# yundantianchang/OpenHyperFLOW2D

Measured on AMD Instinct MI355X. Metric: Mcells·iters/sec (whole node) on Wedge15 2000×200, higher is better.
Workload: dtype fp64

## Files before the change

openhyperflow2d_amd/csrc/bind/module.cpp:

```cpp
#include <algorithm>
#include <pybind11/functional.h>
#include <pybind11/numpy.h>
#include <pybind11/pybind11.h>
#include <pybind11/stl.h>

#include <cstring>
#include <iostream>
#include <sstream>

#include "../core/case.hpp"
#include "../core/checkpoint.hpp"
#include "../core/lean_euler.hpp"
#include "../core/postproc.hpp"
#include "../core/solver.hpp"
#include "../hip/chem_mech.hpp"
#include "../hip/chem_fast.hpp"
#include "../hip/chem_rtc.hpp"
#include "../hip/device_solver.hpp"
#include "../hip/numerics.hpp"

namespace py = pybind11;
using namespace hf2d;

namespace {
// ... 487 lines not shown
            const CellRecord& n = c.J.at(i, j);
            double v;
            if (name == "p_total") v = p_asterisk(n);
            else if (name == "T_total") v = T_asterisk(n);
            else if (name == "schlieren") v = schlieren(n);
            else throw std::runtime_error("unknown derived field " + name);
            m(i, j) = v;
          }
        return a;
      })
      .def("save_heat_flux", [](const Case& c, const std::string& px, const std::string& py_) {
        need_whole(c);
        if (!px.empty()) save_x_heat_flux(px, c, c.J);
        if (!py_.empty()) save_y_heat_flux(py_, c, c.J);
      });

  m.def(
      "lean_tile_geom",
      [](int ncols, int ny, int block, int tj, int cpt) {
        const LeanTile T = lean_tile_geom(ncols, ny, block, tj, cpt);
        py::dict d;
        d["TI"] = T.TI;
        d["TJ"] = T.TJ;
        d["W"] = T.W;
        d["NC"] = T.NC;
        d["nbi"] = T.nbi;
        d["nbj"] = T.nbj;
        d["TIh"] = T.TIh;
        d["CPT"] = T.CPT;
        return d;
      },
      py::arg("ncols"), py::arg("ny"), py::arg("block"), py::arg("tj") = 0, py::arg("cpt") = 1,
      "lean tile geometry (lean_euler.hpp LeanTile) of a strip of ncols x ny cells");
  m.def("sk_eligible", [](const Case& c) { std::string w; const int md = sk_eligible(c, &w); return py::make_tuple(md, w); },
        py::arg("case"), "split-kernel specialisation (0 generic, 1 single-gas laminar, 2 single-gas turbulent; reason)");
  m.def("smooth", [](py::array_t<double, py::array::c_style> a, int axis) {
        if (a.ndim() != 2) throw std::runtime_error("smooth: (nx, ny) array expected");
        auto buf = a.mutable_data();
        if (axis == 0) smooth_x(buf, (int)a.shape(0), (int)a.shape(1));
        else smooth_y(buf, (int)a.shape(0), (int)a.shape(1));
      }, py::arg("a"), py::arg("axis"), "SmoothX (axis 0) / SmoothY (axis 1), in place");
  m.def("cond_names", &cond_names, py::arg("CT"), "PrintCond: names of the set CondType2D bits");
  m.def("turb_cond_names", &turb_cond_names, py::arg("TT"), "PrintTurbCond: names of the set TurbulenceCondType2D bits");

  py::class_<SolverBase>(m, "SolverBase")
      .def("run_steps", &SolverBase::run_steps, py::arg("n"), py::arg("want_residual_last") = false,
           py::call_guard<py::gil_scoped_release>())
      .def("advance", [](SolverBase& s, bool want) { s.advance(want); }, py::arg("want_residual") = false)
      .def_property_readonly("phase_times",
                             [](const SolverBase& s) {
                               py::dict d;
                               for (const auto& kv : s.phase_acc)
                                 d[py::str(kv.first)] = py::make_tuple(kv.second.first, kv.second.second);
                               return d;
                             })
      .def("set_comm",
           [](SolverBase& s, int rank, int size, std::function<double(double)> fmin, std::function<double(double)> fsum,
              std::function<int(int)> fmaxi, std::function<py::bytes(py::bytes)> fres,
              std::function<py::object(py::bytes)> fallgather) {
             auto* c = new PyComm();
             c->r = rank;
             c->n = size;
             c->f_min = fmin;
             c->f_sum = fsum;
             c->f_maxi = fmaxi;
             c->f_res = fres;
// ... 368 lines not shown
      .def_readonly("gi0", &DeviceSolver::gi0)
      .def_readonly("gi1", &DeviceSolver::gi1)
      .def_property(
          "lnm_phase_ms",
          [](const DeviceSolver& s) {
            return std::vector<double>(s.lnm_phase_ms, s.lnm_phase_ms + 4);
          },
          [](DeviceSolver& s, const std::vector<double>& v) {
            for (int q = 0; q < 4; q++) s.lnm_phase_ms[q] = q < (int)v.size() ? v[q] : 0.0;
          })
      .def("lnm_trace_fetch", &DeviceSolver::lnm_trace_fetch, py::call_guard<py::gil_scoped_release>())
      .def("comm_rank", &DeviceSolver::comm_rank)
      .def("comm_size", &DeviceSolver::comm_size)
      .def("synchronize", &DeviceSolver::synchronize, py::call_guard<py::gil_scoped_release>())
      .def("autotune", &DeviceSolver::autotune, py::arg("steps") = 120, py::call_guard<py::gil_scoped_release>())
      .def("trace_tile", &DeviceSolver::trace_tile, py::arg("steps") = 20,
           "one phase-traced lean tile step: per workgroup [entry, staged, wave0 computed, reduced, dt atomic done "
           "(s_memrealtime, 100 MHz), HW_ID, XCC_ID, blockIdx]")
      .def_property_readonly("lean_tile_last",
                             [](const DeviceSolver& s) {
                               const DeviceSolver::TileLast& t = s.lean_tile_last;
                               py::dict d;
                               d["nt"] = t.nt;
                               d["cpt"] = t.cpt;
                               d["TI"] = t.TI;
                               d["TJ"] = t.TJ;
                               d["nbi"] = t.nbi;
                               d["nbj"] = t.nbj;
                               d["stagger"] = t.stagger;
                               d["fx"] = t.fx;
                               d["var"] = t.var;
                               d["seen"] = t.seen;
                               d["dt_read"] = t.dt_read;
                               return d;
                             },
                             "geometry and variant (0 plain, 1 outputs, 2 residual) of the last lean tile launch; "
                             "nt == 0 after a step on any other kernel")
      .def("halo_field_count", [](const DeviceSolver& d, int group, bool full) {
        std::vector<real*> f;
        d.halo_fields(group, f, full);
        return (int)f.size();
      }, py::arg("group"), py::arg("full") = false)
      .def_property("lean_plain", [](const DeviceSolver& d) { return d.lean_plain; },
                    [](DeviceSolver& d, bool on) { d.set_lean_plain(on); })
      .def_property_readonly("stream", [](const DeviceSolver& s) { return (uintptr_t)s.stream(); });
}
```

openhyperflow2d_amd/csrc/core/lean_euler.hpp:

```cpp
#pragma once

#include <algorithm>
#include <cstring>

#include "stepkern.hpp"

namespace hf2d {

HF_HD inline bool same_bits(real a, real b) {
  u64 x, y;
  std::memcpy(&x, &a, sizeof x);
  std::memcpy(&y, &b, sizeof y);
  return x == y;
}

enum : uint8_t { LB_DX_OUT = 16, LB_DY_OUT = 32, LB_PLAIN = 64 };

struct LeanSoA {
  long N = 0;
  const real* Sin;
  real* Sout;
  const real* Pin_s;
  real* Pout_s;
  real* beta;
// ... 37 lines not shown
  const long N = L.N;
  switch (k) {
    case I_RHO: return L.Sin[2 * N + at];
    case I_RHOU: return L.Sin[2 * N + at] * u;
    case I_RHOV: return p + L.Sin[2 * N + at] * v;
    case I_RHOE: return (L.Sin[3 * N + at] + p) * v;
    default: return L.Pin_s[(k - 4) * N + at] * v;
  }
}

struct LeanOwn {
  u64 CT = 0;
  uint8_t lb = 0;
  bool filled = false;
  real beta[4 + NCOMP];
  real CP = 0, R = 0, kk = 0;
};

template <int NE = 4 + NCOMP>
HF_HD inline void lean_load_own(const LeanSoA& L, long idx, LeanOwn& o) {
  const long N = L.N;
  o.CT = L.CT[idx];
  o.lb = L.lb[idx];
  o.filled = !has_all(o.CT, CT_SOLID) && has_all(o.CT, CT_NODE_IS_SET);
  if (o.filled) {
#pragma unroll
    for (int k = 0; k < NE; k++) o.beta[k] = L.beta[k * N + idx];
    o.CP = L.CP[idx];
    o.R = L.R[idx];
    o.kk = L.kk[idx];
  }
}

struct LeanIOCommon {
  static constexpr int NE = 4 + NCOMP;
  static constexpr bool skip(int) { return false; }
  HF_HD static constexpr int eq(int k) { return k; }
  const LeanSoA& L;
  long N, idx, iL, iR, iU, iD;
  uint8_t lb = 0;
  bool noslip = false;
  real FT = 0;
  const real* obeta = nullptr;
  bool skip_same = false;
  real sm[NEQ];

  HF_HD LeanIOCommon(const LeanSoA& l, long i) : L(l), N(l.N), idx(i), iL(i), iR(i), iU(i), iD(i) {}
  HF_HD void set_nb_global(int i, int j, int ny, int n1, int n2, int n3, int n4) {
    iL = (long)(i - n1) * ny + j;
    iR = (long)(i + n2) * ny + j;
    iU = idx + n3;
    iD = idx - n4;
  }
  HF_HD real dxL(int k) const { return L.dSdx_in[k * N + iL]; }
  HF_HD real dxR(int k) const { return L.dSdx_in[k * N + iR]; }
  HF_HD real dyU(int k) const { return L.dSdy_in[k * N + iU]; }
  HF_HD real dyD(int k) const { return L.dSdy_in[k * N + iD]; }
  HF_HD real beta(int k) const { return obeta[k]; }
  HF_HD real Src(int) const { return 0.0; }
  HF_HD real SrcAdd(int k) const { return noslip ? L.SrcAdd[k * N + idx] : 0.0; }
  HF_HD void put_S(int k, real v) { sm[k] = v; }
  HF_HD void put_beta(int k, real v) const {
    if (!skip_same || !same_bits(v, obeta[k])) L.beta[k * N + idx] = v;
  }
  HF_HD void put_dS(int k, real a, real b) const {
    if (lb & LB_DX_OUT) L.dSdx_out[k * N + idx] = a;
// ... 194 lines not shown
        c.Tf = L.Tf[idx];
        c.CT = CT;
        c.lam = c.mu = 0.;
        if (SG)
          chemistry_single_gas(c, *P.species);
        else
          chemistry_zeldovich(c, *P.species, P.sm, P.chem_model);
        if (c.R != own.R) io.out_R(c.R);
        if (!io.skip_same || !same_bits(c.CP, own.CP)) io.out_CP(c.CP);
        if (OUT || noslip)
          for (int q = 0; q < NSPEC; q++) L.Y[q * N + idx] = c.Y[q];
      }
    }
  }
  for (int k = 0; k < NE; k++) io.out_S(k, s[k]);
  io.out_UVP(U, V, p);
  if (OUT) {
    L.Tout[idx] = Tg;
    L.kk[idx] = kk;
  }
  return dt_local;
}

constexpr int LEAN_TILE_FIELDS = 13;
constexpr int LEAN_TILE_FIELDS_SG = 7;
inline int lean_tile_fields(bool sg) { return sg ? LEAN_TILE_FIELDS_SG : LEAN_TILE_FIELDS; }
constexpr int LEAN_TILE_MIN_TJ = 8;

struct LeanTile {
  int TI, TJ, W, NC, nbi, nbj;
  int TIh;
  int CPT;
  int ne = 1;
};

inline LeanTile lean_tile_geom(int ncols, int ny, int block, int tj = 0, int cpt = 1) {
  LeanTile T;
  if (tj > 0) {
    T.TJ = std::min(std::max(tj, LEAN_TILE_MIN_TJ), std::min(block, ny));
  } else if (ny <= 32) {
    T.TJ = ny;
  } else {
    double best = -1;
    T.TJ = 32;
    for (int c = 16; c <= 32; c++) {
      const int nj = (ny + c - 1) / c;
      const double eff = (double)((block / c) * c) / block * (double)ny / (nj * c);
      if (eff > best + 1e-12) {
        best = eff;
        T.TJ = c;
      }
    }
  }
  T.CPT = cpt;
  T.TIh = block / T.TJ;
  T.TI = T.TIh * cpt;
  T.W = T.TJ + 2;
  T.NC = (T.TI + 2) * T.W;
  T.nbi = (ncols + T.TI - 1) / T.TI;
  T.nbj = (ny + T.TJ - 1) / T.TJ;
  return T;
}

template <bool SG = false>
HF_HD inline void lean_tile_stage(const StepParams& P, const LeanSoA& L, const LeanTile& T, int i0, int j0,
                                  real* lds, int t, int nthreads) {
// ... 146 lines not shown
```

openhyperflow2d_amd/csrc/hip/dev_common.hpp:

```cpp
#pragma once

#include <hip/hip_runtime.h>

#include "../core/lean_euler.hpp"
#include "../core/stepkern.hpp"

namespace hf2d {

struct DevScalars {
  unsigned long long dt_bits[3];
  double iter[3];
  double beta_min[3], cfl_min[3];
  double time_part;
  int neg_T;
  int pad;
  double dt_val[3];
  unsigned hot_cnt[3];
  unsigned hot_cnt2[3];
  unsigned long long dt_lag[3];
  alignas(128) unsigned long long dt_sh[3][16][16];
};
constexpr int DT_SHARDS = 16;

__device__ inline double bits_to_d(unsigned long long b) { return __longlong_as_double((long long)b); }
// ... 43 lines not shown
  else if (lane == DT_SHARDS) b = sc->dt_bits[slot];
#pragma unroll
  for (int off = 1; off < 32; off <<= 1) b = dt_bits_min(b, (unsigned long long)__shfl_xor((long long)b, off, 64));
  return bits_to_d((unsigned long long)__shfl((long long)b, 0, 64));
}

__device__ inline double dt_cur(const StepParams& P, const DevScalars* sc, int slot) {
  return __builtin_expect(P.lag_dt != 0, 0) ? bits_to_d(sc->dt_lag[slot]) : dt_get(sc, slot);
}
__device__ inline double dt_cur_tile(const StepParams& P, const DevScalars* sc, int slot) {
  if (__builtin_expect(P.lag_dt != 0, 0)) return bits_to_d(sc->dt_lag[slot]);
  if (P.dt_read == 2) return bits_to_d(sc->dt_bits[slot]);
  if (P.dt_read == 1) return dt_get_wave(sc, slot);
  return dt_get(sc, slot);
}
__device__ inline void lag_head(const StepParams& P, DevScalars* sc, int slot, int slot_next, double fold = 1.0) {
  if (P.lag_dt) {
    const double m = dt_get(sc, slot);
    sc->dt_lag[slot_next] = d_to_bits(fold < m ? fold : m);
  }
}

__device__ inline void apply_dt(StepParams& P, const DevScalars* sc, int slot, bool tile = false) {
  const double dt = tile ? dt_cur_tile(P, sc, slot) : dt_cur(P, sc, slot);
  P.dt = dt;
  P.dtdx = dt / P.dx;
  P.dtdy = dt / P.dy;
  if (P.scen) {
    P.beta_min = sc->beta_min[slot];
    P.CFL_min = sc->cfl_min[slot];
  }
}

__device__ inline void scenario_next(const StepParams& P, DevScalars* sc, int slot, int slot_next) {
  const double it = sc->iter[slot] + 1.0;
  sc->iter[slot_next] = it;
  if (P.scen) {
    const real bs = table_eval(P.scen->beta, it), cs = table_eval(P.scen->cfl, it);
    sc->beta_min[slot_next] = (bs < P.scen->beta0) ? bs : P.scen->beta0;
    sc->cfl_min[slot_next] = (cs < P.scen->CFL) ? cs : P.scen->CFL;
  }
}

constexpr int BLOCK = 256;
constexpr int WAVE = 64;

__device__ inline void shfl_merge(ResidualPack& r, int off) {
#pragma unroll
  for (int k = 0; k < NEQ; k++) {
    EqResidual o;
    o.dd_max = __shfl_xor(r.eq[k].dd_max, off, WAVE);
    o.i = __shfl_xor(r.eq[k].i, off, WAVE);
    o.j = __shfl_xor(r.eq[k].j, off, WAVE);
    o.rms = __shfl_xor(r.eq[k].rms, off, WAVE);
    o.sum_div = __shfl_xor(r.eq[k].sum_div, off, WAVE);
    o.count = __shfl_xor(r.eq[k].count, off, WAVE);
    EqResidual& f = r.eq[k];
    const bool later = (o.i > f.i) || (o.i == f.i && o.j > f.j);
    if (o.dd_max > f.dd_max || (o.dd_max == f.dd_max && later)) {
      f.dd_max = o.dd_max;
      f.i = o.i;
      f.j = o.j;
    }
    f.rms += o.rms;
    f.sum_div += o.sum_div;
    f.count += o.count;
// ... 6 lines not shown
  if (b >= q * NUM_XCD) return b;
  return (b % NUM_XCD) * q + b / NUM_XCD;
}

constexpr int MAX_HALO_FIELDS = 128;
struct ColList {
  real* f[MAX_HALO_FIELDS];
  unsigned char o[MAX_HALO_FIELDS] = {};
  int nf;
};
constexpr long P2P_SPIN_LIMIT = 1L << 26;
constexpr int P2P_THREADS = 512;

__device__ inline unsigned long long p2p_acquire(const unsigned long long* f) {
  return __hip_atomic_load(f, __ATOMIC_ACQUIRE, __HIP_MEMORY_SCOPE_SYSTEM);
}

__device__ inline double p2p_load(const double* p) {
  return __longlong_as_double((long long)__hip_atomic_load((const unsigned long long*)p, __ATOMIC_RELAXED,
                                                           __HIP_MEMORY_SCOPE_SYSTEM));
}
__device__ inline float p2p_load(const float* p) {
  return __int_as_float((int)__hip_atomic_load((const unsigned*)p, __ATOMIC_RELAXED, __HIP_MEMORY_SCOPE_SYSTEM));
}

__device__ inline void p2p_store(double* p, double v) {
  __hip_atomic_store((unsigned long long*)p, (unsigned long long)__double_as_longlong(v), __ATOMIC_RELAXED,
                     __HIP_MEMORY_SCOPE_SYSTEM);
}
__device__ inline void p2p_store(float* p, float v) {
  __hip_atomic_store((unsigned*)p, (unsigned)__float_as_int(v), __ATOMIC_RELAXED, __HIP_MEMORY_SCOPE_SYSTEM);
}
__device__ inline void vm_drain() { asm volatile("s_waitcnt vmcnt(0)" ::: "memory"); }

__device__ inline unsigned long long rt_clock() { return __builtin_amdgcn_s_memrealtime(); }
constexpr int FX_DONE_STRIDE = 32;
constexpr int FX_TRACE_N = 64, FX_TRACE_W = 8;
constexpr unsigned FX_COUNT1_MAX = 512;
constexpr int FX_DONE_WORDS = (DT_SHARDS + 1) * FX_DONE_STRIDE + 2 * FX_TRACE_N * FX_TRACE_W;
struct FusedX {
  real* peer_recv_l;
  real* peer_recv_r;
  const real* my_recv;
  unsigned long long* const* peer_flags;
  double* const* peer_dtr;
  const unsigned long long* my_flags;
  const double* my_dtr;
  unsigned long long* seq;
  unsigned* done;
  long cap;
  int rank, nranks, sides, on;
  int defer;
  int skip;
  int edge_first;
  int count1;
};

__device__ inline double wave_min(double v) {
#pragma unroll
  for (int off = 1; off < WAVE; off <<= 1) v = fmin(v, __shfl_xor(v, off, WAVE));
  return v;
}
template <class Need>
__device__ inline double p2p_wait_wave(const FusedX& x, unsigned long long target, DevScalars* sc, Need need,
                                       bool fold, int par, bool* ok) {
  const int lane = (int)(threadIdx.x & (WAVE - 1));
// ... 164 lines not shown
```

openhyperflow2d_amd/csrc/hip/device_solver.hpp:

```cpp
#pragma once

#include <algorithm>
#include <chrono>
#include <condition_variable>
#include <cstdlib>
#include <memory>
#include <mutex>
#include <string>
#include <thread>
#include <vector>

#include "../core/solver.hpp"
#include "device_knobs.hpp"

namespace hf2d {

struct LnmArrays;
struct LeanTile;

bool gpu_available();

struct LocalGroup {
  explicit LocalGroup(int n_)
      : n(n_), send_l(n_), send_r(n_), dt_src(n_, nullptr), vals(n_), packs(n_), blobs(n_) {
    const char* j = std::getenv("HF2D_LOCAL_JITTER_US");
    jitter_us = j ? std::max(0, std::atoi(j)) : 0;
  }
  int n;
  std::mutex mu;
  std::condition_variable cv;
  int arrived = 0;
  long gen = 0;
  int jitter_us = 0;
  unsigned long long jitter_state = 0x9E3779B97F4A7C15ull;
  void jitter() {
    unsigned long long x;
    {
      std::lock_guard<std::mutex> lk(mu);
      jitter_state ^= jitter_state << 13;
      jitter_state ^= jitter_state >> 7;
      jitter_state ^= jitter_state << 17;
      x = jitter_state;
    }
    std::this_thread::sleep_for(std::chrono::microseconds((long)(x % (unsigned long long)jitter_us)));
  }
  std::vector<real*> send_l, send_r;
  std::vector<const unsigned long long*> dt_src;
  std::vector<double> vals;
  std::vector<ResidualPack> packs;
  std::vector<std::string> blobs;
  void barrier() {
    if (jitter_us > 0) jitter();
    std::unique_lock<std::mutex> lk(mu);
// ... 67 lines not shown
  void halo_fields(int group, std::vector<real*>& f, bool full = false) const;
  void halo_fields(int group, std::vector<real*>& f, std::vector<unsigned char>& o, bool full) const;
  std::string p2p_probe();
  std::vector<unsigned long long> fx_trace();
  static bool p2p_probe_ok(const std::vector<std::string>& blobs, int rank, std::string* why);
  void p2p_fallback();

  std::vector<unsigned long long> lnm_trace_fetch();
  void set_lean_plain(bool on);
  void lean_materialize();
  void lns_materialize();
  void flush_pending();

  bool lean_ok = false;
  std::string lean_why;
  bool lean_sg_ok = false;
  bool lean_has_cauchy_x = true;
  bool any_cauchy_x = true;
  bool sgl_ok = false;
  std::string sgl_why;
  int sk_mode = 0;
  bool lns_ok = false;
  std::string lns_why;
  int lns_turb = 2;
  bool lnm_ok = false;
  std::string lnm_why;
  int lnm_turb = 0;
  bool chem_fast_ok = false;
  bool chem_rtc_ok = false;
  std::string chem_rtc_why;
  std::string chem_kernel_used;
  struct TileLast {
    int nt = 0, cpt = 0, TI = 0, TJ = 0, nbi = 0, nbj = 0, stagger = 0, fx = 0, var = 0, seen = 0, dt_read = 0;
  };
  TileLast lean_tile_last;

  long nstep = 0;
  long lns_steps = 0, lnm_steps = 0;
  long lns_fx_steps = 0;
  long lns_prologue_steps = 0;
  long p2p_mwg_exchanges = 0;
  long overlap_steps = 0;
  long graph_launches = 0;
  long graph_captures = 0;
  double lnm_phase_ms[4] = {0, 0, 0, 0};

  HostArrays h;
  int dev = 0;
  int gi0 = 0, gi1 = 0, l_off = 0;
  int abuf = 0, dsbuf = 0, pbuf = 0, sbuf = 0;
  int cbuf = 0;
  int lean_state = 0;
  int lns_state = 0;
  bool lean_plain = false;
  bool lean_T_stored = true;
  int lns_prev_mu_t = -1;
  double time_offset = 0.0, last_dev_time = 0.0;
  bool dt_word_valid = false;
  unsigned long long* tile_trace = nullptr;
  std::vector<long> probe_idx_host;
  std::vector<real> probe_buf_host;
  int probe_gen = 0;
  long probe_cap = 0;
  std::vector<long> probe_rec_idx;
  bool stats_on = false;
  bool stats_armed = false;
// ... 69 lines not shown
```

openhyperflow2d_amd/csrc/hip/lean_tile.hpp:

```cpp
#pragma once

#include "../core/lean_euler.hpp"
#include "dev_common.hpp"

namespace hf2d {

__device__ __forceinline__ void host_mirror_tail(const StepParams& P, DevScalars* sc, int slot_next) {
  const int lane = (int)(threadIdx.x & (WAVE - 1));
  vm_drain();
  int last = 0;
  if (lane == 0) {
    const unsigned G = gridDim.x, sh = blockIdx.x % DT_SHARDS;
    const unsigned pop = (G - sh + DT_SHARDS - 1) / DT_SHARDS, nsh = G < DT_SHARDS ? G : DT_SHARDS;
    unsigned* cs = P.host_done + sh * FX_DONE_STRIDE;
    unsigned* ct = P.host_done + DT_SHARDS * FX_DONE_STRIDE;
    if (__hip_atomic_fetch_add(cs, 1u, __ATOMIC_RELAXED, __HIP_MEMORY_SCOPE_AGENT) == pop - 1) {
      __hip_atomic_store(cs, 0u, __ATOMIC_RELAXED, __HIP_MEMORY_SCOPE_AGENT);
      if (__hip_atomic_fetch_add(ct, 1u, __ATOMIC_RELAXED, __HIP_MEMORY_SCOPE_AGENT) == nsh - 1) {
        __hip_atomic_store(ct, 0u, __ATOMIC_RELAXED, __HIP_MEMORY_SCOPE_AGENT);
        last = 1;
      }
    }
  }
  if (!__shfl(last, 0, WAVE)) return;
  unsigned long long b = ~0ull;
  if (lane < DT_SHARDS) b = __hip_atomic_load(&sc->dt_sh[slot_next][lane][0], __ATOMIC_RELAXED, __HIP_MEMORY_SCOPE_AGENT);
  if (lane == DT_SHARDS) b = __hip_atomic_load(&sc->dt_bits[slot_next], __ATOMIC_RELAXED, __HIP_MEMORY_SCOPE_AGENT);
  if (P.dt_fold) {
    unsigned long long m = b;
#pragma unroll
    for (int off = 1; off < 32; off <<= 1) m = dt_bits_min(m, (unsigned long long)__shfl_xor((long long)m, off, WAVE));
    m = (unsigned long long)__shfl((long long)m, 0, WAVE);
    if (lane == DT_SHARDS) {
      b = m;
      __hip_atomic_store(&sc->dt_bits[slot_next], m, __ATOMIC_RELAXED, __HIP_MEMORY_SCOPE_AGENT);
    }
  }
  if (!P.host_sc) return;
  DevScalars* h = static_cast<DevScalars*>(P.host_sc);
  if (lane <= DT_SHARDS) (lane < DT_SHARDS ? h->dt_sh[slot_next][lane][0] : h->dt_bits[slot_next]) = b;
  if (lane == DT_SHARDS + 1) h->neg_T = __hip_atomic_load(&sc->neg_T, __ATOMIC_RELAXED, __HIP_MEMORY_SCOPE_AGENT);
}
__device__ __forceinline__ void host_mirror_head(const StepParams& P, const DevScalars* sc, int slot_next) {
  DevScalars* h = static_cast<DevScalars*>(P.host_sc);
  h->time_part = sc->time_part;
  h->dt_lag[slot_next] = sc->dt_lag[slot_next];
}

constexpr int TILE_TRACE_WORDS = 8;
#ifndef HF2D_TILE_STAGGER
#define HF2D_TILE_STAGGER 1
#endif
constexpr int LDS_PER_CU = 160 * 1024;


template <bool RES, bool OUT, bool SG, int CPT, bool FX = false, bool TR = false, int NT = BLOCK>
__device__ __forceinline__ void lean_tile_body(StepParams& P, const LeanSoA& L, const LeanTile& T, DevScalars* sc,
                                               int slot, int slot_next, int serial, ResidualPack* partials,
                                               const FusedX& X = FusedX{}, unsigned long long* trace = nullptr,
                                               int part = 0) {
  extern __shared__ real lds[];
  unsigned long long tr[5];
  if (TR) tr[0] = rt_clock();
  if (HF2D_TILE_STAGGER && SG && CPT == 2 && !FX && NT == BLOCK && P.stagger != 0) {
    const unsigned r = blockIdx.x / (unsigned)P.stagger_wgs;
    if (r < 4 && (P.stagger < 0 || r > 0)) {
      const unsigned long long d = P.stagger > 0 ? (unsigned long long)r * (unsigned)P.stagger
                                                 : (unsigned long long)blockIdx.x * (unsigned)(-P.stagger) /
                                                       (unsigned)P.stagger_wgs;
      const unsigned long long t0 = rt_clock();
      while (rt_clock() - t0 < d) __builtin_amdgcn_s_sleep(2);
    }
  }
  const unsigned b = (FX && X.edge_first) ? tile_edge_first(xcd_remap(blockIdx.x, gridDim.x), T)
                                          : tile_of_part(xcd_remap(blockIdx.x, gridDim.x), part, T);
  unsigned long long seq_prev = 0;
  if (FX) seq_prev = *X.seq;
  apply_dt(P, sc, slot, true);
  if (b == 0 && threadIdx.x < WAVE) {
    double fold = 1.0;
    if (FX && X.defer && P.lag_dt && seq_prev > 0) {
      bool ok;
      fold = p2p_wait_wave(X, seq_prev, sc, [](int) { return true; }, true, (int)(seq_prev & 1), &ok);
    }
    if (threadIdx.x == 0) {
      dt_reset(sc, slot_reset(slot));
      lag_head(P, sc, slot, slot_next, fold);
      sc->dt_bits[slot] = d_to_bits(P.dt);
      sc->time_part += P.dt;
      scenario_next(P, sc, slot, slot_next);
      if (OUT && !RES && !FX && P.host_sc) host_mirror_head(P, sc, slot_next);
    }
  }
  int i[CPT], j[CPT], c[CPT], i0, j0;
  bool mine[CPT];
  LeanOwn own[CPT];
#pragma unroll
  for (int q = 0; q < CPT; q++) {
    mine[q] = lean_tile_cell(P, T, (int)b, (int)threadIdx.x, &i[q], &j[q], &c[q], &i0, &j0, q);
    if (mine[q]) lean_load_own<TileIO<SG>::NE>(L, (long)i[q] * P.ny + j[q], own[q]);
  }
  if (!FX || seq_prev == 0 || (X.skip & 4) || (i0 - 1 > P.i0 - 1 && i0 + T.TI < P.i1)) {
    lean_tile_stage<SG>(P, L, T, i0, j0, lds, threadIdx.x, NT);
  } else {
    constexpr int NF = SG ? LEAN_TILE_FIELDS_SG : LEAN_TILE_FIELDS;
    const int pp = (int)(seq_prev & 1);
    const real* mbL = X.my_recv + ((long)pp * 2) * X.cap;
    const real* mbR = X.my_recv + ((long)pp * 2 + 1) * X.cap;
    const long N = L.N;
    constexpr int NS = SG ? 4 : 4 + NCOMP;
    constexpr int FU = SG ? 4 : 10;
    for (int c = threadIdx.x; c < T.NC; c += NT) {
      const int ii = c / T.W - 1, jj = c - (ii + 1) * T.W - 1;
      const bool xh = ii < 0 || ii >= T.TI, yh = jj < 0 || jj >= T.TJ;
      const int gi = i0 + ii, gj = j0 + jj;
      if ((xh && yh) || gi < 0 || gi >= P.nx || gj < 0 || gj >= P.ny) continue;
      const bool gl = (X.sides & 1) && gi == P.i0 - 1, gr = (X.sides & 2) && gi == P.i1;
      if (gl || gr) {
        const real* mb = gl ? mbL : mbR;
#pragma unroll
        for (int f = 0; f < NF; f++) lds[f * T.NC + c] = p2p_load(mb + (long)f * P.ny + gj);
        continue;
      }
      const long g = (long)gi * P.ny + gj;
#pragma unroll
      for (int f = 0; f < NS; f++) lds[f * T.NC + c] = L.Sin[f * N + g];
      if (!SG)
#pragma unroll
        for (int f = 0; f < NCOMP; f++) lds[(4 + NCOMP + f) * T.NC + c] = L.Pin_s[f * N + g];
      lds[FU * T.NC + c] = L.Uin[g];
      lds[(FU + 1) * T.NC + c] = L.Vin[g];
      lds[(FU + 2) * T.NC + c] = L.Pin[g];
    }
  }
  __syncthreads();
  if (TR) tr[1] = rt_clock();
  ResidualPack r;
  if (RES) {
    residual_reset(r);
#pragma unroll
    for (int k = 0; k < NEQ; k++) r.eq[k].i = r.eq[k].j = -1;
  }
  double dtl = 1.0;
  int neg = 0;
#pragma unroll
  for (int q = 0; q < CPT; q++) {
    if (mine[q]) {
      TileIO<SG> io(L, (long)i[q] * P.ny + j[q], lds, T.NC, T.W, c[q]);
      dtl = fmin(dtl, lean_cell<RES, OUT>(P, L, io, own[q], i[q], j[q], r, &neg));
      if (FX) {
        const bool pl = (X.sides & 1) && i[q] == P.i0, pr = (X.sides & 2) && i[q] == P.i1 - 1;
        if ((pl || pr) && !(X.skip & 2)) {
          constexpr int NF = SG ? LEAN_TILE_FIELDS_SG : LEAN_TILE_FIELDS;
          constexpr int NS = SG ? 4 : 4 + NCOMP;
          const int pn = (int)((seq_prev + 1) & 1);
          real* mb = pl ? X.peer_recv_l + ((long)pn * 2 + 1) * X.cap : X.peer_recv_r + ((long)pn * 2) * X.cap;
          const long N = L.N, g = (long)i[q] * P.ny + j[q];
          real v[NF];
#pragma unroll
          for (int f = 0; f < NS; f++) v[f] = L.Sout[f * N + g];
          if (!SG)
#pragma unroll
            for (int f = 0; f < NCOMP; f++) v[4 + NCOMP + f] = L.Pout_s[f * N + g];
          v[NF - 3] = L.Uout[g];
          v[NF - 2] = L.Vout[g];
          v[NF - 1] = L.Pout[g];
#pragma unroll
          for (int f = 0; f < NF; f++) p2p_store(mb + (long)f * P.ny + j[q], v[f]);
// ... 84 lines not shown
```

openhyperflow2d_amd/csrc/hip/step_tile.hip:

```cpp

#include "device_impl.hpp"
#include "lean_tile.hpp"

namespace hf2d {

template <bool RES, bool FROMG>
__global__ __launch_bounds__(BLOCK) void hf2d_lean_euler(StepParams P, LeanSoA L, long c0, long c1, DevScalars* sc,
                                                          int slot, int slot_next, int serial,
                                                          ResidualPack* partials) {
  apply_dt(P, sc, slot);
  const unsigned b = xcd_remap(blockIdx.x, gridDim.x);
  const long g = (long)b * BLOCK + threadIdx.x;
  if (g == 0) {
    dt_reset(sc, slot_reset(slot));
    lag_head(P, sc, slot, slot_next);
    sc->dt_bits[slot] = d_to_bits(P.dt);
    sc->time_part += P.dt;
    scenario_next(P, sc, slot, slot_next);
  }
  const long c = c0 + g;
  ResidualPack r;
  if (RES) {
    residual_reset(r);
#pragma unroll
// ... 45 lines not shown
     {hf2d_lean_tile<false, false, true, 0, 2>, hf2d_lean_tile<false, true, true, 0, 2>,
      hf2d_lean_tile<true, true, true, 0, 2>}}};
static const TileFxK kTileFx[2][2][3] = {
    {{hf2d_lean_tile_fx<false, false, false, 1>, hf2d_lean_tile_fx<false, true, false, 1>,
      hf2d_lean_tile_fx<true, true, false, 1>},
     {hf2d_lean_tile_fx<false, false, false, 2>, hf2d_lean_tile_fx<false, true, false, 2>,
      hf2d_lean_tile_fx<true, true, false, 2>}},
    {{hf2d_lean_tile_fx<false, false, true, 1>, hf2d_lean_tile_fx<false, true, true, 1>,
      hf2d_lean_tile_fx<true, true, true, 1>},
     {hf2d_lean_tile_fx<false, false, true, 2>, hf2d_lean_tile_fx<false, true, true, 2>,
      hf2d_lean_tile_fx<true, true, true, 2>}}};
static const TileTrK kTileTr[2][2] = {{hf2d_lean_tile_tr<false, 1>, hf2d_lean_tile_tr<false, 2>},
                                      {hf2d_lean_tile_tr<true, 1>, hf2d_lean_tile_tr<true, 2>}};
#define HF2D_NT_ROW(K, NT, CPT) {K<false, false, NT, CPT>, K<false, true, NT, CPT>, K<true, true, NT, CPT>}
static const TileK kTileNt[2][2][3] = {{HF2D_NT_ROW(hf2d_lean_tile_nt, 128, 1), HF2D_NT_ROW(hf2d_lean_tile_nt, 128, 2)},
                                       {HF2D_NT_ROW(hf2d_lean_tile_nt, 64, 1), HF2D_NT_ROW(hf2d_lean_tile_nt, 64, 2)}};
static const TileFxK kTileFxNt[2][2][3] = {
    {HF2D_NT_ROW(hf2d_lean_tile_fx_nt, 128, 1), HF2D_NT_ROW(hf2d_lean_tile_fx_nt, 128, 2)},
    {HF2D_NT_ROW(hf2d_lean_tile_fx_nt, 64, 1), HF2D_NT_ROW(hf2d_lean_tile_fx_nt, 64, 2)}};
#undef HF2D_NT_ROW
static const TileTrK kTileTrNt[2][2] = {{hf2d_lean_tile_tr_nt<128, 1>, hf2d_lean_tile_tr_nt<128, 2>},
                                        {hf2d_lean_tile_tr_nt<64, 1>, hf2d_lean_tile_tr_nt<64, 2>}};
inline int tile_nt(int want, bool sg) { return sg && (want == 128 || want == 64) ? want : BLOCK; }
inline TileK tile_kernel(int nt, bool sg, int cpt, int var) {
  return nt == BLOCK ? kTile[sg][cpt - 1][var] : kTileNt[nt == 128 ? 0 : 1][cpt - 1][var];
}
inline TileFxK tile_fx_kernel(int nt, bool sg, int cpt, int var) {
  return nt == BLOCK ? kTileFx[sg][cpt - 1][var] : kTileFxNt[nt == 128 ? 0 : 1][cpt - 1][var];
}
inline TileTrK tile_tr_kernel(int nt, bool sg, int cpt) {
  return nt == BLOCK ? kTileTr[sg][cpt - 1] : kTileTrNt[nt == 128 ? 0 : 1][cpt - 1];
}

using LeanEulerK = void (*)(StepParams, LeanSoA, long, long, DevScalars*, int, int, int, ResidualPack*);
static const LeanEulerK kLeanEuler[2][2] = {{hf2d_lean_euler<false, false>, hf2d_lean_euler<false, true>},
                                            {hf2d_lean_euler<true, false>, hf2d_lean_euler<true, true>}};

void DeviceSolver::lean_materialize() {
  p2p_complete();
  Impl& m = *impl;
  StepParams P = make_params(last_iter + iter);
  P.nx = h.nx;
  P.ny = h.ny;
  LeanSoA L = m.lean_view(h, sbuf, abuf, dsbuf, pbuf, false);
  SoA g = m.view(h, sbuf, abuf, dsbuf, pbuf);
  const unsigned nb = (unsigned)((h.N + BLOCK - 1) / BLOCK);
  hipLaunchKernelGGL(hf2d_lean_materialize, dim3(nb), dim3(BLOCK), 0, m.stream, P, L, g, 0L, h.N);
  HIP_CHECK(hipGetLastError());
  lean_state = 0;
}

DeviceSolver::StepDone DeviceSolver::step_tile(StepCtx& c) {
  Impl& m = *impl;
  hipStream_t st = m.stream;
  StepParams& P = c.P;
  const bool want_res = c.want_res;
  const int slot = c.slot, slot_next = c.slot_next, serial = c.serial;
  LeanSoA L = m.lean_view(h, sbuf, abuf, dsbuf, pbuf, false);
  P.skip_same = tile_skip_same ? 1 : 0;
  P.dt_read = dt_read_mode == 1 ? 1 : 0;
  const bool sg = lean_sg && lean_sg_ok;
  const int nt = tile_nt(lean_nt, sg);
  int cpt = lean_cpt == 2 ? 2 : 1;
  if (cpt == 2 && nt == BLOCK) {
    const LeanTile T2 = lean_tile_geom(P.i1 - P.i0, P.ny, BLOCK, lean_tj, 2);
    if ((long)T2.nbi * T2.nbj < 2L * cu_count) cpt = 1;
  }
  const LeanTile T = lean_tile_geom(P.i1 - P.i0, P.ny, nt, lean_tj, cpt);
  const unsigned ntile = (unsigned)(T.nbi * T.nbj);
  size_t shmem = (size_t)lean_tile_fields(sg) * T.NC * sizeof(real);
  if (lean_wgcu > 0)
    shmem = std::max(shmem, (size_t)((LDS_PER_CU / lean_wgcu - 1024) & ~255));
  const bool rec_out = (probe_cap > 0 || stats_on) && !sg && P.chem_model != NO_REACTIONS;
  const bool out = step_outputs || want_res || rec_out;
  P.stagger_wgs = cu_count > 0 ? cu_count : 256;
  P.stagger = ntile <= 4u * (unsigned)P.stagger_wgs && nt == BLOCK ? tile_stagger : 0;
  const bool fx_step = m.p2p.on && p2p_fuse && !lean_has_cauchy_x;
  FusedX X = fx_step ? fused_args() : FusedX{};
  X.defer = fx_step && P.lag_dt ? 1 : 0;
  lean_tile_last.nt = nt;
  lean_tile_last.cpt = cpt;
  lean_tile_last.TI = T.TI;
  lean_tile_last.TJ = T.TJ;
  lean_tile_last.nbi = T.nbi;
  lean_tile_last.nbj = T.nbj;
  lean_tile_last.stagger = HF2D_TILE_STAGGER && sg && cpt == 2 && !fx_step && nt == BLOCK ? P.stagger : 0;
  lean_tile_last.fx = fx_step ? 1 : 0;
  lean_tile_last.seen = c.tile_prev.nt == nt && c.tile_prev.cpt == cpt ? c.tile_prev.seen : 0;
  const bool split = comm_overlap && !fx_step && !m.p2p.on && (m.comm || m.local) && m.nranks > 1 &&
                     !want_res && !out && !tile_trace;
  if (split) {
    lean_tile_last.seen |= 1;
    lean_T_stored = false;
    overlap_streams();
    const bool parts = T.nbi >= 3;
    const unsigned ne = parts ? (unsigned)(2 * T.nbj) : ntile, ni = parts ? (unsigned)((T.nbi - 2) * T.nbj) : 0u;
    const TileK pk = tile_kernel(nt, sg, cpt, 0);
    hipLaunchKernelGGL(pk, dim3(ne), dim3(nt), shmem, st, P, L, T, m.sc, slot, slot_next, serial, m.partials,
                       parts ? 1 : 0);
    HIP_CHECK(hipGetLastError());
    sbuf = 1 - sbuf;
    dsbuf = 1 - dsbuf;
    pbuf = 1 - pbuf;
    HIP_CHECK(hipEventRecord(m.ev_edge, st));
    if (ni > 0)
      hipLaunchKernelGGL(pk, dim3(ni), dim3(nt), shmem, st, P, L, T, m.sc, slot, slot_next, serial, m.partials,
                         2);
    HIP_CHECK(hipGetLastError());
    overlap_exchange(CpuSolver::HALO_LEAN, slot_next);
    return {ntile, nt / WAVE, true};
  }
  const int var = want_res ? 2 : out ? 1 : 0;
  lean_tile_last.var = var;
  lean_tile_last.seen |= 1 << var;
  lean_T_stored = var != 0;
  if (tile_trace && var == 0 && !fx_step)
    hipLaunchKernelGGL(tile_tr_kernel(nt, sg, cpt), dim3(ntile), dim3(nt), shmem, st, P, L, T, m.sc, slot, slot_next,
                       serial, m.partials, tile_trace);
// ... 77 lines not shown
```

Measured before the change: 14270.

## Batch single-gas tile halo loads in registers and defer dt/wg0 head past staging

For the single-gas lean tile kernel, the tile halo staging becomes a batch that issues all global loads for up to three slots per thread into registers first. The own-cell beta/CP/R/kk loads and the dt reduction are interleaved with those loads, and only then are the values written to LDS, so memory latency overlaps instead of serialising. The dt read is split into an issue phase and a finish phase, and workgroup 0's head bookkeeping moves after the __syncthreads. The cost is higher register pressure from holding 21 doubles per thread, which may lower occupancy, and the reordered dt/head logic is a correctness risk.

```diff
diff --git a/openhyperflow2d_amd/csrc/bind/module.cpp b/openhyperflow2d_amd/csrc/bind/module.cpp
--- a/openhyperflow2d_amd/csrc/bind/module.cpp
+++ b/openhyperflow2d_amd/csrc/bind/module.cpp
@@ -543,6 +543,9 @@
       },
       py::arg("ncols"), py::arg("ny"), py::arg("block"), py::arg("tj") = 0, py::arg("cpt") = 1,
       "lean tile geometry (lean_euler.hpp LeanTile) of a strip of ncols x ny cells");
+  m.def("lean_tile_stage_kmax", &lean_tile_stage_kmax, py::arg("nt"), py::arg("cpt"),
+        "largest slots per thread (ceil(NC / nt)) the single-gas lean tile kernel stages in one batch of loads; "
+        "beyond it the kernel runs the staging loop (lean_tile_last['stage'] == 0)");
   m.def("sk_eligible", [](const Case& c) { std::string w; const int md = sk_eligible(c, &w); return py::make_tuple(md, w); },
         py::arg("case"), "split-kernel specialisation (0 generic, 1 single-gas laminar, 2 single-gas turbulent; reason)");
   m.def("smooth", [](py::array_t<double, py::array::c_style> a, int axis) {
@@ -977,6 +980,7 @@
                                d["var"] = t.var;
                                d["seen"] = t.seen;
                                d["dt_read"] = t.dt_read;
+                               d["stage"] = t.stage;
                                return d;
                              },
                              "geometry and variant (0 plain, 1 outputs, 2 residual) of the last lean tile launch; "
diff --git a/openhyperflow2d_amd/csrc/core/lean_euler.hpp b/openhyperflow2d_amd/csrc/core/lean_euler.hpp
--- a/openhyperflow2d_amd/csrc/core/lean_euler.hpp
+++ b/openhyperflow2d_amd/csrc/core/lean_euler.hpp
@@ -93,6 +93,23 @@
   }
 }
 
+HF_HD inline void lean_load_own_flags(const LeanSoA& L, long idx, LeanOwn& o) {
+  o.CT = L.CT[idx];
+  o.lb = L.lb[idx];
+}
+template <int NE = 4 + NCOMP>
+HF_HD inline void lean_load_own_rest(const LeanSoA& L, long idx, LeanOwn& o) {
+  const long N = L.N;
+  o.filled = !has_all(o.CT, CT_SOLID) && has_all(o.CT, CT_NODE_IS_SET);
+  if (o.filled) {
+#pragma unroll
+    for (int k = 0; k < NE; k++) o.beta[k] = L.beta[k * N + idx];
+    o.CP = L.CP[idx];
+    o.R = L.R[idx];
+    o.kk = L.kk[idx];
+  }
+}
+
 struct LeanIOCommon {
   static constexpr int NE = 4 + NCOMP;
   static constexpr bool skip(int) { return false; }
@@ -353,6 +370,7 @@
   int TIh;
   int CPT;
   int ne = 1;
+  int stage = 0;
 };
 
 inline LeanTile lean_tile_geom(int ncols, int ny, int block, int tj = 0, int cpt = 1) {
diff --git a/openhyperflow2d_amd/csrc/hip/dev_common.hpp b/openhyperflow2d_amd/csrc/hip/dev_common.hpp
--- a/openhyperflow2d_amd/csrc/hip/dev_common.hpp
+++ b/openhyperflow2d_amd/csrc/hip/dev_common.hpp
@@ -99,6 +99,34 @@
   }
 }
 
+__device__ inline unsigned long long dt_tile_issue(StepParams& P, const DevScalars* sc, int slot) {
+  if (P.scen) {
+    P.beta_min = sc->beta_min[slot];
+    P.CFL_min = sc->cfl_min[slot];
+  }
+  if (__builtin_expect(P.lag_dt != 0, 0)) return sc->dt_lag[slot];
+  if (P.dt_read == 2) return sc->dt_bits[slot];
+  if (P.dt_read == 1) {
+    const int lane = (int)(threadIdx.x & 63);
+    unsigned long long b = ~0ull;
+    if (lane < DT_SHARDS) b = sc->dt_sh[slot][lane][0];
+    else if (lane == DT_SHARDS) b = sc->dt_bits[slot];
+    return b;
+  }
+  return d_to_bits(dt_get(sc, slot));
+}
+__device__ inline void dt_tile_finish(StepParams& P, unsigned long long b) {
+  if (!__builtin_expect(P.lag_dt != 0, 0) && P.dt_read == 1) {
+#pragma unroll
+    for (int off = 1; off < 32; off <<= 1) b = dt_bits_min(b, (unsigned long long)__shfl_xor((long long)b, off, 64));
+    b = (unsigned long long)__shfl((long long)b, 0, 64);
+  }
+  const double dt = bits_to_d(b);
+  P.dt = dt;
+  P.dtdx = dt / P.dx;
+  P.dtdy = dt / P.dy;
+}
+
 __device__ inline void scenario_next(const StepParams& P, DevScalars* sc, int slot, int slot_next) {
   const double it = sc->iter[slot] + 1.0;
   sc->iter[slot_next] = it;
@@ -171,6 +199,8 @@
   __hip_atomic_store((unsigned*)p, (unsigned)__float_as_int(v), __ATOMIC_RELAXED, __HIP_MEMORY_SCOPE_SYSTEM);
 }
 __device__ inline void vm_drain() { asm volatile("s_waitcnt vmcnt(0)" ::: "memory"); }
+
+__device__ inline void keep_whole(u64& v) { asm volatile("" : "+v"(v)); }
 
 __device__ inline unsigned long long rt_clock() { return __builtin_amdgcn_s_memrealtime(); }
 constexpr int FX_DONE_STRIDE = 32;
diff --git a/openhyperflow2d_amd/csrc/hip/device_solver.hpp b/openhyperflow2d_amd/csrc/hip/device_solver.hpp
--- a/openhyperflow2d_amd/csrc/hip/device_solver.hpp
+++ b/openhyperflow2d_amd/csrc/hip/device_solver.hpp
@@ -19,6 +19,7 @@
 struct LeanTile;
 
 bool gpu_available();
+int lean_tile_stage_kmax(int nt, int cpt);
 
 struct LocalGroup {
   explicit LocalGroup(int n_)
@@ -152,6 +153,7 @@
   std::string chem_kernel_used;
   struct TileLast {
     int nt = 0, cpt = 0, TI = 0, TJ = 0, nbi = 0, nbj = 0, stagger = 0, fx = 0, var = 0, seen = 0, dt_read = 0;
+    int stage = 0;
   };
   TileLast lean_tile_last;
 
diff --git a/openhyperflow2d_amd/csrc/hip/lean_tile.hpp b/openhyperflow2d_amd/csrc/hip/lean_tile.hpp
--- a/openhyperflow2d_amd/csrc/hip/lean_tile.hpp
+++ b/openhyperflow2d_amd/csrc/hip/lean_tile.hpp
@@ -53,6 +53,69 @@
 #endif
 constexpr int LDS_PER_CU = 160 * 1024;
 
+__host__ __device__ constexpr int lean_stage_kmax(int nt, int cpt) {
+  (void)nt;
+  (void)cpt;
+  return 3;
+}
+constexpr int LEAN_STAGE_KTOP = 3;
+template <int KM>
+struct LeanStaged {
+  real v[KM > 0 ? KM : 1][LEAN_TILE_FIELDS_SG];
+  int c[KM > 0 ? KM : 1];
+};
+template <int K, int NT, int KM>
+__device__ __forceinline__ void lean_stage_issue(const StepParams& P, const LeanSoA& L, const LeanTile& T, int i0,
+                                                 int j0, LeanStaged<KM>& s) {
+  static_assert(K <= KM, "slots");
+  const long N = L.N;
+#pragma unroll
+  for (int k = 0; k < K; k++) {
+    const int c = (int)threadIdx.x + k * NT;
+    const int ii = c / T.W - 1, jj = c - (ii + 1) * T.W - 1;
+    const bool xh = ii < 0 || ii >= T.TI, yh = jj < 0 || jj >= T.TJ;
+    const int gi = i0 + ii, gj = j0 + jj;
+    const bool skip = c >= T.NC || (xh && yh) || gi < 0 || gi >= P.nx || gj < 0 || gj >= P.ny;
+    s.c[k] = skip ? -1 : c;
+    if (!skip) {
+      const long g = (long)gi * P.ny + gj;
+#pragma unroll
+      for (int f = 0; f < 4; f++) s.v[k][f] = L.Sin[f * N + g];
+      s.v[k][4] = L.Uin[g];
+      s.v[k][5] = L.Vin[g];
+      s.v[k][6] = L.Pin[g];
+    }
+  }
+}
+template <int K, int KM>
+__device__ __forceinline__ void lean_stage_write(const LeanTile& T, const LeanStaged<KM>& s, real* lds) {
+  static_assert(K <= KM, "slots");
+#pragma unroll
+  for (int k = 0; k < K; k++)
+    if (s.c[k] >= 0)
+#pragma unroll
+      for (int f = 0; f < LEAN_TILE_FIELDS_SG; f++) lds[f * T.NC + s.c[k]] = s.v[k][f];
+}
+
+template <bool MIRROR, bool FX>
+__device__ __forceinline__ void lean_tile_wg0_head(const StepParams& P, DevScalars* sc, int slot, int slot_next,
+                                                   const FusedX& X, unsigned long long seq_prev) {
+  if (threadIdx.x < WAVE) {
+    double fold = 1.0;
+    if (FX && X.defer && P.lag_dt && seq_prev > 0) {
+      bool ok;
+      fold = p2p_wait_wave(X, seq_prev, sc, [](int) { return true; }, true, (int)(seq_prev & 1), &ok);
+    }
+    if (threadIdx.x == 0) {
+      dt_reset(sc, slot_reset(slot));
+      lag_head(P, sc, slot, slot_next, fold);
+      sc->dt_bits[slot] = d_to_bits(P.dt);
+      sc->time_part += P.dt;
+      scenario_next(P, sc, slot, slot_next);
+      if (MIRROR && P.host_sc) host_mirror_head(P, sc, slot_next);
+    }
+  }
+}
 
 template <bool RES, bool OUT, bool SG, int CPT, bool FX = false, bool TR = false, int NT = BLOCK>
 __device__ __forceinline__ void lean_tile_body(StepParams& P, const LeanSoA& L, const LeanTile& T, DevScalars* sc,
@@ -76,33 +139,47 @@
                                           : tile_of_part(xcd_remap(blockIdx.x, gridDim.x), part, T);
   unsigned long long seq_prev = 0;
   if (FX) seq_prev = *X.seq;
-  apply_dt(P, sc, slot, true);
-  if (b == 0 && threadIdx.x < WAVE) {
-    double fold = 1.0;
-    if (FX && X.defer && P.lag_dt && seq_prev > 0) {
-      bool ok;
-      fold = p2p_wait_wave(X, seq_prev, sc, [](int) { return true; }, true, (int)(seq_prev & 1), &ok);
-    }
-    if (threadIdx.x == 0) {
-      dt_reset(sc, slot_reset(slot));
-      lag_head(P, sc, slot, slot_next, fold);
-      sc->dt_bits[slot] = d_to_bits(P.dt);
-      sc->time_part += P.dt;
-      scenario_next(P, sc, slot, slot_next);
-      if (OUT && !RES && !FX && P.host_sc) host_mirror_head(P, sc, slot_next);
-    }
-  }
+  unsigned long long dtb = 0;
+  if (SG) dtb = dt_tile_issue(P, sc, slot);
+  else apply_dt(P, sc, slot, true);
+  if (!SG && b == 0) lean_tile_wg0_head<OUT && !RES && !FX, FX>(P, sc, slot, slot_next, X, seq_prev);
   int i[CPT], j[CPT], c[CPT], i0, j0;
   bool mine[CPT];
   LeanOwn own[CPT];
 #pragma unroll
   for (int q = 0; q < CPT; q++) {
     mine[q] = lean_tile_cell(P, T, (int)b, (int)threadIdx.x, &i[q], &j[q], &c[q], &i0, &j0, q);
-    if (mine[q]) lean_load_own<TileIO<SG>::NE>(L, (long)i[q] * P.ny + j[q], own[q]);
-  }
-  if (!FX || seq_prev == 0 || (X.skip & 4) || (i0 - 1 > P.i0 - 1 && i0 + T.TI < P.i1)) {
+    if (mine[q]) {
+      if (SG) lean_load_own_flags(L, (long)i[q] * P.ny + j[q], own[q]);
+      else lean_load_own<TileIO<SG>::NE>(L, (long)i[q] * P.ny + j[q], own[q]);
+    }
+  }
+  const bool plain = !FX || seq_prev == 0 || (X.skip & 4) || (i0 - 1 > P.i0 - 1 && i0 + T.TI < P.i1);
+  if (SG && plain) {
+    constexpr int KMAX = lean_stage_kmax(NT, CPT);
+    static_assert(KMAX <= LEAN_STAGE_KTOP, "lean_tile_body dispatches K <= LEAN_STAGE_KTOP");
+    LeanStaged<KMAX> s;
+    const int K = T.stage;
+    if (KMAX >= 2 && K == 2) lean_stage_issue<(KMAX >= 2 ? 2 : 0), NT>(P, L, T, i0, j0, s);
+    else if (KMAX >= 3 && K == 3) lean_stage_issue<(KMAX >= 3 ? 3 : 0), NT>(P, L, T, i0, j0, s);
+#pragma unroll
+    for (int q = 0; q < CPT; q++) {
+      keep_whole(own[q].CT);
+      if (mine[q]) lean_load_own_rest<4>(L, (long)i[q] * P.ny + j[q], own[q]);
+    }
+    dt_tile_finish(P, dtb);
+    if (KMAX >= 2 && K == 2) lean_stage_write<(KMAX >= 2 ? 2 : 0)>(T, s, lds);
+    else if (KMAX >= 3 && K == 3) lean_stage_write<(KMAX >= 3 ? 3 : 0)>(T, s, lds);
+    else lean_tile_stage<true>(P, L, T, i0, j0, lds, threadIdx.x, NT);
+  } else if (plain) {
     lean_tile_stage<SG>(P, L, T, i0, j0, lds, threadIdx.x, NT);
   } else {
+    if (SG) {
+#pragma unroll
+      for (int q = 0; q < CPT; q++)
+        if (mine[q]) lean_load_own_rest<4>(L, (long)i[q] * P.ny + j[q], own[q]);
+      dt_tile_finish(P, dtb);
+    }
     constexpr int NF = SG ? LEAN_TILE_FIELDS_SG : LEAN_TILE_FIELDS;
     const int pp = (int)(seq_prev & 1);
     const real* mbL = X.my_recv + ((long)pp * 2) * X.cap;
@@ -134,6 +211,7 @@
     }
   }
   __syncthreads();
+  if (SG && b == 0) lean_tile_wg0_head<OUT && !RES && !FX, FX>(P, sc, slot, slot_next, X, seq_prev);
   if (TR) tr[1] = rt_clock();
   ResidualPack r;
   if (RES) {
diff --git a/openhyperflow2d_amd/csrc/hip/step_tile.hip b/openhyperflow2d_amd/csrc/hip/step_tile.hip
--- a/openhyperflow2d_amd/csrc/hip/step_tile.hip
+++ b/openhyperflow2d_amd/csrc/hip/step_tile.hip
@@ -101,7 +101,15 @@
   return nt == BLOCK ? kTileTr[sg][cpt - 1] : kTileTrNt[nt == 128 ? 0 : 1][cpt - 1];
 }
 
-using LeanEulerK = void (*)(StepParams, LeanSoA, long, long, DevScalars*, int, int, int, ResidualPack*);
+inline int tile_stage_k(const LeanTile& T, int nt, int cpt) {
+  const int K = (T.NC + nt - 1) / nt;
+  return K <= lean_stage_kmax(nt, cpt) ? K : 0;
+}
+int lean_tile_stage_kmax(int nt, int cpt) {
+  return (nt == BLOCK || nt == 128 || nt == 64) && (cpt == 1 || cpt == 2) ? lean_stage_kmax(nt, cpt) : 0;
+}
+
+using LeanEulerK =void (*)(StepParams, LeanSoA, long, long, DevScalars*, int, int, int, ResidualPack*);
 static const LeanEulerK kLeanEuler[2][2] = {{hf2d_lean_euler<false, false>, hf2d_lean_euler<false, true>},
                                             {hf2d_lean_euler<true, false>, hf2d_lean_euler<true, true>}};
 
@@ -135,7 +143,8 @@
     const LeanTile T2 = lean_tile_geom(P.i1 - P.i0, P.ny, BLOCK, lean_tj, 2);
     if ((long)T2.nbi * T2.nbj < 2L * cu_count) cpt = 1;
   }
-  const LeanTile T = lean_tile_geom(P.i1 - P.i0, P.ny, nt, lean_tj, cpt);
+  LeanTile T = lean_tile_geom(P.i1 - P.i0, P.ny, nt, lean_tj, cpt);
+  T.stage = sg ? tile_stage_k(T, nt, cpt) : 0;
   const unsigned ntile = (unsigned)(T.nbi * T.nbj);
   size_t shmem = (size_t)lean_tile_fields(sg) * T.NC * sizeof(real);
   if (lean_wgcu > 0)
@@ -153,6 +162,7 @@
   lean_tile_last.TJ = T.TJ;
   lean_tile_last.nbi = T.nbi;
   lean_tile_last.nbj = T.nbj;
+  lean_tile_last.stage = T.stage;
   lean_tile_last.stagger = HF2D_TILE_STAGGER && sg && cpt == 2 && !fx_step && nt == BLOCK ? P.stagger : 0;
   lean_tile_last.fx = fx_step ? 1 : 0;
   lean_tile_last.seen = c.tile_prev.nt == nt && c.tile_prev.cpt == cpt ? c.tile_prev.seen : 0;
```

After: 15020, median of 6. 1.05x the previous value.
